# haoyu94/RoITr

Hardware: AMD Instinct MI355X
Metric: point-cloud pairs/s (higher is better)
Workload: dtype f32

## Files before the change

roitr_amd/csrc/pointops_knn.hip:

```cpp
#include "common.h"
#include "knn_grid.h"
#include "prof.h"
#include "roitr_pointops.h"
#include <math.h>
#include <stdio.h>
#include <stdlib.h>
#include <type_traits>

#define KNN_FILL 1e10f

namespace {

__device__ __forceinline__ float rl_f(float v, int lane) { return __int_as_float(__builtin_amdgcn_readlane(__float_as_int(v), lane)); }
__device__ __forceinline__ int rl_i(int v, int lane) { return __builtin_amdgcn_readlane(v, lane); }
__device__ __forceinline__ void lds_sync_wave() { asm volatile("s_waitcnt lgkmcnt(0)" ::: "memory"); }
__device__ __forceinline__ void push_query(int* count, int* list, int q) { list[atomicAdd(count, 1)] = q; }

__device__ __forceinline__ void home_cell(const RoitrGrid& g, float x, float y, float z, int (&c)[3])
{
    c[0] = (int)fminf(fmaxf((x - g.ox) * g.inv_h, 0.f), (float)(g.nx - 1));
    c[1] = (int)fminf(fmaxf((y - g.oy) * g.inv_h, 0.f), (float)(g.ny - 1));
    c[2] = (int)fminf(fmaxf((z - g.oz) * g.inv_h, 0.f), (float)(g.nz - 1));
}
struct ShellBox { int x0, x1, y0, y1, z0, z1; };
// ... 88 lines not shown
        const int p = lane + 64 * r;
        if (p < nsample) {
            if (o.idx) o.idx[(size_t)q * nsample + p] = i[r];
            if (o.dist2) o.dist2[(size_t)q * nsample + p] = d[r];
            if (p >= 1) {
                if (o.group_idx) o.group_idx[(size_t)q * (nsample - 1) + p - 1] = i[r];
                if (o.ppf) {
                    const float* pp = xyz + (size_t)i[r] * 3;
                    const float* pn = o.ref_normals + (size_t)i[r] * 3;
                    const float* qn = o.query_normals + (size_t)q * 3;
                    const float4 f = ppf4(Q.x, Q.y, Q.z, qn[0], qn[1], qn[2], pp[0], pp[1], pp[2], pn[0], pn[1], pn[2]);
                    reinterpret_cast<float4*>(o.ppf)[(size_t)q * (nsample - 1) + p - 1] = f;
                }
            }
        }
    }
}

template <int NR>
__device__ __forceinline__ bool has_tie(const WaveList<NR>& L, int nsample, int lane)
{
    bool t = false;
    float nxt_first = 0.f;
    if (NR > 1) nxt_first = rl_f(L.d[NR - 1], 0);
#pragma unroll
    for (int r = 0; r < NR; ++r) {
        float nx = __shfl_down(L.d[r], 1, 64);
        const int p = lane + 64 * r;
        if (lane == 63) nx = (r + 1 < NR) ? nxt_first : __int_as_float(0x7fc00000);
        t |= (p < nsample) && (L.d[r] == nx) && (L.d[r] < KNN_FILL);
    }
    return __ballot(t) != 0ull;
}

__device__ __forceinline__ void find_segment(int q, const int* __restrict__ offset, const int* __restrict__ new_offset, int& start,
                                             int& end, int& seg, int b = 0)
{
    int bt = 0;
    if (b > 0) bt = segment_of(q, new_offset, b);
    else
    while (!(q < new_offset[bt])) bt++;
    start = bt == 0 ? 0 : offset[bt - 1];
    end = offset[bt];
    seg = bt;
}

template <int NR>
__device__ __forceinline__ void finish_query(WaveList<NR>& L, const KnnOut& o, int q, int nsample, int lane, const float* xyz, Query Q)
{
    if (has_tie(L, nsample, lane)) {
        if (lane == 0) push_query(o.tie_count, o.tie_list, q);
        return;
    }
    write_rows<NR>(o, q, nsample, L.d, L.i, lane, xyz, Q);
}

template <int NR>
__global__ __launch_bounds__(256) void knn_brute_kernel(int m, int nsample, const float* __restrict__ xyz,
                                                        const float* __restrict__ new_xyz, const int* __restrict__ offset,
                                                        const int* __restrict__ new_offset, KnnOut o)
{
    const int lane = threadIdx.x & 63;
    const int q = blockIdx.x * 4 + (threadIdx.x >> 6);
    if (q >= m) return;
    int start, end, seg;
    find_segment(q, offset, new_offset, start, end, seg, o.b);
    Query Q = {new_xyz[(size_t)q * 3], new_xyz[(size_t)q * 3 + 1], new_xyz[(size_t)q * 3 + 2]};
    WaveList<NR> L;
    L.init(start);
    const int tau_pos = nsample;
    float tau = KNN_FILL;
    for (int base = start; base < end; base += 64) {
        const int k = base + lane;
        float cd = INFINITY;
        if (k < end) {
            const float* p = xyz + (size_t)k * 3;
            cd = sqdist3(Q.x, Q.y, Q.z, p[0], p[1], p[2]);
        }
        consume_batch<NR>(L, cd, k, tau, tau_pos, lane);
    }
    finish_query<NR>(L, o, q, nsample, lane, xyz, Q);
}

template <int CAP>
__global__ __launch_bounds__(1024) void grid_build_kernel(const float* __restrict__ xyz, const int* __restrict__ offset,
                                                          RoitrGrid* __restrict__ grids, int* __restrict__ cell_start,
                                                          float4* __restrict__ sorted, float target_occupancy)
{
    __shared__ int cnt[CAP];
    __shared__ float red[6][16];
    __shared__ RoitrGrid G;
    __shared__ int wave_tot[16];
    const int c = blockIdx.x;
    const int start = c == 0 ? 0 : offset[c - 1];
    const int end = offset[c];
    const int n = end - start;
    const int tid = threadIdx.x, lane = tid & 63, wave = tid >> 6;
    int* cs = cell_start + (size_t)c * (GRID_MAX_CELLS + 1);

    float mn[3] = {INFINITY, INFINITY, INFINITY}, mx[3] = {-INFINITY, -INFINITY, -INFINITY};
    for (int k = start + tid; k < end; k += 1024) {
#pragma unroll
        for (int a = 0; a < 3; ++a) {
            const float v = xyz[(size_t)k * 3 + a];
            mn[a] = fminf(mn[a], v); mx[a] = fmaxf(mx[a], v);
        }
    }
#pragma unroll
    for (int a = 0; a < 3; ++a) {
        const float lo = -wave_max(-mn[a]), hi = wave_max(mx[a]);
        if (lane == 0) { red[a][wave] = lo; red[3 + a][wave] = hi; }
    }
    __shared__ int occ_cells;
    __shared__ int refine;
    if (tid == 0) occ_cells = 0;
    __syncthreads();
    auto choose = [&](float h_want) {
        float lo[3], ext[3], me = 0.f;
        for (int a = 0; a < 3; ++a) {
            float l = red[a][0], h = red[3 + a][0];
            for (int w = 1; w < 16; ++w) { l = fminf(l, red[a][w]); h = fmaxf(h, red[3 + a][w]); }
            if (n == 0) { l = 0.f; h = 0.f; }
            lo[a] = l; ext[a] = h - l; me = fmaxf(me, ext[a]);
        }
        if (!(me > 0.f)) me = 1.f;
        float h = h_want;
        if (!(h > 0.f)) {
            float vol = 1.f;
            for (int a = 0; a < 3; ++a) vol *= fmaxf(ext[a], 1e-3f * me);
            h = cbrtf(vol * target_occupancy / (float)(n > 0 ? n : 1));
        }
        h = fmaxf(h, me / (float)GRID_MAX_DIM);
        int d[3];
        for (;;) {
            long tot = 1;
            for (int a = 0; a < 3; ++a) {
                int v = (int)floorf(ext[a] / h) + 1;
                d[a] = v < 1 ? 1 : (v > GRID_MAX_DIM ? GRID_MAX_DIM : v);
                tot *= d[a];
            }
            if (tot <= CAP) break;
            h *= 1.26f;
        }
        G.ox = lo[0]; G.oy = lo[1]; G.oz = lo[2]; G.h = h; G.inv_h = 1.0f / h; G.nx = d[0]; G.ny = d[1]; G.nz = d[2];
    };
    if (tid == 0) choose(0.f);
    __syncthreads();
    for (int k = tid; k < G.nx * G.ny * G.nz; k += 1024) cnt[k] = 0;
    __syncthreads();
    auto cell_of_g = [&](float x, float y, float z) {
        int cx = (int)floorf((x - G.ox) * G.inv_h), cy = (int)floorf((y - G.oy) * G.inv_h), cz = (int)floorf((z - G.oz) * G.inv_h);
        cx = min(max(cx, 0), G.nx - 1); cy = min(max(cy, 0), G.ny - 1); cz = min(max(cz, 0), G.nz - 1);
        return (cz * G.ny + cy) * G.nx + cx;
    };
    for (int pass = 0; pass < 3; ++pass) {
        for (int k = start + tid; k < end; k += 1024)
            atomicAdd(&cnt[cell_of_g(xyz[(size_t)k * 3], xyz[(size_t)k * 3 + 1], xyz[(size_t)k * 3 + 2])], 1);
        __syncthreads();
        if (pass == 2) break;
        const int nc_ = G.nx * G.ny * G.nz;
        int occ_l = 0;
        for (int k = tid; k < nc_; k += 1024) occ_l += cnt[k] > 0 ? 1 : 0;
        occ_l = (int)wave_sum((float)occ_l);
        if (lane == 0 && occ_l) atomicAdd(&occ_cells, occ_l);
        __syncthreads();
        if (tid == 0) {
            const float have = (float)n / (float)max(occ_cells, 1);
            refine = 0;
            if (n > 0 && have > 1.3f * target_occupancy) {
                const float h_old = G.h;
                choose(h_old * cbrtf(target_occupancy / have));
                refine = G.h < 0.97f * h_old ? 1 : 0;
                if (!refine) choose(h_old);
            }
            occ_cells = 0;
        }
        __syncthreads();
        if (!refine) break;
        for (int k = tid; k < G.nx * G.ny * G.nz; k += 1024) cnt[k] = 0;
        __syncthreads();
    }
    if (tid == 0) grids[c] = G;
    const RoitrGrid g = G;
    const int ncell = g.nx * g.ny * g.nz;
    auto cell_of = [&](float x, float y, float z) {
        int cx = (int)floorf((x - g.ox) * g.inv_h), cy = (int)floorf((y - g.oy) * g.inv_h), cz = (int)floorf((z - g.oz) * g.inv_h);
        cx = min(max(cx, 0), g.nx - 1); cy = min(max(cy, 0), g.ny - 1); cz = min(max(cz, 0), g.nz - 1);
        return (cz * g.ny + cy) * g.nx + cx;
    };
    {
        constexpr int PER = CAP / 1024;
        int loc[PER], s = 0;
#pragma unroll
        for (int j = 0; j < PER; ++j) { const int k = tid * PER + j; loc[j] = k < ncell ? cnt[k] : 0; s += loc[j]; }
        int incl = s;
#pragma unroll
        for (int o = 1; o < 64; o <<= 1) { const int v = __shfl_up(incl, o, 64); if (lane >= o) incl += v; }
        if (lane == 63) wave_tot[wave] = incl;
        __syncthreads();
        int wbase = 0;
        for (int w = 0; w < wave; ++w) wbase += wave_tot[w];
        int run = wbase + incl - s;
#pragma unroll
        for (int j = 0; j < PER; ++j) {
            const int k = tid * PER + j;
            if (k < ncell) { cnt[k] = run; cs[k] = start + run; }
            run += loc[j];
        }
        if (tid == 0) cs[ncell] = start + n;
    }
    __syncthreads();
    for (int k = start + tid; k < end; k += 1024) {
        const float x = xyz[(size_t)k * 3], y = xyz[(size_t)k * 3 + 1], z = xyz[(size_t)k * 3 + 2];
        const int pos = atomicAdd(&cnt[cell_of(x, y, z)], 1);
        sorted[start + pos] = make_float4(x, y, z, __int_as_float(k));
    }
}

constexpr int SEL_CAP = 1024;

template <int J>
__device__ __forceinline__ int lane_xor(int v, int lane)
{
    if (J == 1) return __builtin_amdgcn_update_dpp(0, v, 0xB1, 0xf, 0xf, true);
    if (J == 2) return __builtin_amdgcn_update_dpp(0, v, 0x4E, 0xf, 0xf, true);
    if (J == 4) {
        const int dn = __builtin_amdgcn_update_dpp(0, v, 0x124, 0xf, 0xa, false);
        return __builtin_amdgcn_update_dpp(dn, v, 0x12C, 0xf, 0x5, false);
    }
    if (J == 8) return __builtin_amdgcn_update_dpp(0, v, 0x128, 0xf, 0xf, true);
    return __shfl_xor(v, J, 64);
}

template <int K, int J>
__device__ __forceinline__ void sort128_step(WaveList<2>& L, int lane)
{
#pragma unroll
    for (int r = 0; r < 2; ++r) {
        const int e = lane + 64 * r;
        const float pd = __int_as_float(lane_xor<J>(__float_as_int(L.d[r]), lane));
        const int pi = lane_xor<J>(L.i[r], lane);
        const bool up = (e & K) == 0;
        const bool lower = (lane & J) == 0;
        const unsigned long long mk_ = ((unsigned long long)__float_as_uint(L.d[r]) << 32) | (unsigned)L.i[r];
        const unsigned long long pk_ = ((unsigned long long)__float_as_uint(pd) << 32) | (unsigned)pi;
        const bool mine_gt = mk_ > pk_;
        const bool take = (lower == up) ? mine_gt : !mine_gt;
        L.d[r] = take ? pd : L.d[r];
        L.i[r] = take ? pi : L.i[r];
    }
}
template <int K>
__device__ __forceinline__ void sort128_stage(WaveList<2>& L, int lane)
{
    if (K >= 128) {
        const bool sw = (L.d[0] > L.d[1]) || (L.d[0] == L.d[1] && L.i[0] > L.i[1]);
        const float td = sw ? L.d[1] : L.d[0]; const int ti = sw ? L.i[1] : L.i[0];
        L.d[1] = sw ? L.d[0] : L.d[1]; L.i[1] = sw ? L.i[0] : L.i[1];
        L.d[0] = td; L.i[0] = ti;
    }
    if (K >= 64) sort128_step<K, 32>(L, lane);
    if (K >= 32) sort128_step<K, 16>(L, lane);
    if (K >= 16) sort128_step<K, 8>(L, lane);
    if (K >= 8) sort128_step<K, 4>(L, lane);
    if (K >= 4) sort128_step<K, 2>(L, lane);
    sort128_step<K, 1>(L, lane);
}
__device__ __forceinline__ void wave_sort128(WaveList<2>& L, int lane)
{
    sort128_stage<2>(L, lane); sort128_stage<4>(L, lane); sort128_stage<8>(L, lane); sort128_stage<16>(L, lane);
    sort128_stage<32>(L, lane); sort128_stage<64>(L, lane); sort128_stage<128>(L, lane);
}
__global__ __launch_bounds__(256) void knn_gridsel_kernel(int m, int nsample, const float* __restrict__ xyz,
                                                          const float* __restrict__ new_xyz, const int* __restrict__ offset,
                                                          const int* __restrict__ new_offset, const RoitrGrid* __restrict__ grids,
                                                          const int* __restrict__ cell_start, const float4* __restrict__ sorted, KnnOut o,
                                                          const int* __restrict__ qlist, const int* __restrict__ qcount)
{
    __shared__ float bd_[4][SEL_CAP];
    __shared__ int bi_[4][SEL_CAP];
    __shared__ float ld_[4][128];
    __shared__ int li_[4][128];
    __shared__ int hist_[4][64];
    const int lane = threadIdx.x & 63, w = threadIdx.x >> 6;
    const int n_q = qlist ? *qcount : m;
    for (int t_ = blockIdx.x * 4 + w; t_ < n_q; t_ += gridDim.x * 4) {
    const int q = qlist ? qlist[t_] : t_;
    float* bd = bd_[w]; int* bi = bi_[w]; float* ld = ld_[w]; int* li = li_[w]; int* hist = hist_[w];
    int start, end, seg;
    find_segment(q, offset, new_offset, start, end, seg, o.b);
    const RoitrGrid g = grids[seg];
    const int* cs = cell_start + (size_t)seg * (GRID_MAX_CELLS + 1);
    Query Q = {new_xyz[(size_t)q * 3], new_xyz[(size_t)q * 3 + 1], new_xyz[(size_t)q * 3 + 2]};
    WaveList<2> L;
    L.init(start);
    const int need = nsample + 1;
    float tau = KNN_FILL;
    int cnt = 0;
    bool overflow = false, sorted_ok = false;
// ... 291 lines not shown
            const int S1 = S + 1;
            const float hi = lim;
            const float scale = 64.0f / hi;
            hist[lane] = 0;
            lds_sync_wave();
            int bin[4];
#pragma unroll
            for (int r = 0; r < 4; ++r) {
                bin[r] = min(63, (int)(e[r] * scale));
                if (lane + 64 * r < cnt) atomicAdd(&hist[bin[r]], 1);
            }
            lds_sync_wave();
            const int h = hist[lane];
            const int incl = wave_incl_scan(h, lane);
            const unsigned long long ge = __ballot(incl >= S1);
            const int B = __ffsll((long long)ge) - 1;
            const int nB = rl_i(h, B);
            const int r_need = S1 - (rl_i(incl, B) - nB);
            float tau;
            {
                int base = 0;
                bool too_many = false;
#pragma unroll
                for (int r = 0; r < 4; ++r) {
                    const bool inb = (lane + 64 * r < cnt) && bin[r] == B;
                    const unsigned long long mk = __ballot(inb);
                    const int pos = __builtin_amdgcn_mbcnt_hi((unsigned)(mk >> 32), __builtin_amdgcn_mbcnt_lo((unsigned)mk, base));
                    if (inb && pos < 64) sd[pos] = e[r];
                    base += __popcll(mk);
                }
                too_many = base > 64;
                if (too_many) { retry(q); continue; }
                lds_sync_wave();
                const float v = lane < nB ? sd[lane] : INFINITY;
                int rank = 0;
                for (int u = 0; u < nB; ++u) rank += (rl_f(v, u) < v) ? 1 : 0;
                const float tv = (lane < nB && rank < r_need) ? v : -1.0f;
                tau = wave_max(tv);
                const int n_le = __popcll(__ballot(lane < nB && v <= tau));
                if (n_le != r_need) { tie(q); continue; }
            }
            {
                int base = 0;
#pragma unroll
                for (int r = 0; r < 4; ++r) {
                    const bool sel = e[r] <= tau && ej[r] != qslot;
                    const unsigned long long mk = __ballot(sel);
                    const int pos = __builtin_amdgcn_mbcnt_hi((unsigned)(mk >> 32), __builtin_amdgcn_mbcnt_lo((unsigned)mk, base));
                    if (sel && pos < 64) { sd[pos] = e[r]; sj[pos] = ej[r]; }
                    base += __popcll(mk);
                }
                if (base != S) { retry(q); continue; }
            }
            lds_sync_wave();
            float d = lane < S ? sd[lane] : INFINITY;
            int j = lane < S ? sj[lane] : 0;
            wave_sort64(d, j, lane);
            {
                const float nxd = __shfl_down(d, 1, 64);
                const bool t = (lane + 1 < S && d == nxd) || (lane == 0 && d == 0.f);
                if (__ballot(t) != 0ull) { tie(q); continue; }
            }
            const float4 nb = j >= 0 ? cand[j] : sorted[-j - 1];
            const int ni = __float_as_int(nb.w);
            if (lane == 0) {
                if (o.idx) o.idx[(size_t)q * nsample] = q;
                if (o.dist2) o.dist2[(size_t)q * nsample] = 0.f;
            }
            if (lane < S) {
                if (o.idx) o.idx[(size_t)q * nsample + lane + 1] = ni;
                if (o.dist2) o.dist2[(size_t)q * nsample + lane + 1] = d;
                if (o.group_idx) o.group_idx[(size_t)q * S + lane] = ni;
                if (o.ppf) {
                    const float* pn = o.ref_normals + (size_t)ni * 3;
                    const float* qn = o.query_normals + (size_t)q * 3;
                    reinterpret_cast<float4*>(o.ppf)[(size_t)q * S + lane] =
                        ppf4(Qp.x, Qp.y, Qp.z, qn[0], qn[1], qn[2], nb.x, nb.y, nb.z, pn[0], pn[1], pn[2]);
                }
            }
        }
    }
}

template <int CAP>
__global__ __launch_bounds__(1024) void sort_queries_kernel(const float* __restrict__ new_xyz, const int* __restrict__ new_offset,
                                                            const RoitrGrid* __restrict__ grids, int* __restrict__ qorder)
{
    __shared__ int cnt[CAP];
    __shared__ int wave_tot[16];
    const int c = blockIdx.x;
    const int start = c == 0 ? 0 : new_offset[c - 1], end = new_offset[c];
    const int tid = threadIdx.x, lane = tid & 63, wave = tid >> 6;
    const RoitrGrid g = grids[c];
    const int ncell = g.nx * g.ny * g.nz;
    auto cell_of = [&](int k) {
        int c0[3];
        home_cell(g, new_xyz[(size_t)k * 3], new_xyz[(size_t)k * 3 + 1], new_xyz[(size_t)k * 3 + 2], c0);
        return (c0[2] * g.ny + c0[1]) * g.nx + c0[0];
    };
    for (int k = tid; k < ncell; k += 1024) cnt[k] = 0;
    __syncthreads();
    for (int k = start + tid; k < end; k += 1024) atomicAdd(&cnt[cell_of(k)], 1);
    __syncthreads();
    constexpr int PER = CAP / 1024;
    int loc[PER], sum = 0;
#pragma unroll
    for (int j = 0; j < PER; ++j) { const int k = tid * PER + j; loc[j] = k < ncell ? cnt[k] : 0; sum += loc[j]; }
    int incl = sum;
#pragma unroll
    for (int o = 1; o < 64; o <<= 1) { const int v = __shfl_up(incl, o, 64); if (lane >= o) incl += v; }
    if (lane == 63) wave_tot[wave] = incl;
    __syncthreads();
    int run = incl - sum;
    for (int w = 0; w < wave; ++w) run += wave_tot[w];
#pragma unroll
    for (int j = 0; j < PER; ++j) { const int k = tid * PER + j; if (k < ncell) cnt[k] = run; run += loc[j]; }
    __syncthreads();
    for (int k = start + tid; k < end; k += 1024) qorder[start + atomicAdd(&cnt[cell_of(k)], 1)] = k;
}

template <int L>
__device__ __forceinline__ void lane_emit(const KnnOut& o, int q, int nsample, const float (&d)[L], const int (&id)[L], bool tie,
                                          const float* __restrict__ xyz, float qx, float qy, float qz)
{
    if (tie) {
        push_query(o.tie_count, o.tie_list, q);
        return;
    }
#pragma unroll
    for (int j = 0; j < L; ++j) {
        if (j < nsample) {
            if (o.idx) o.idx[(size_t)q * nsample + j] = id[j];
            if (o.dist2) o.dist2[(size_t)q * nsample + j] = d[j];
            if (j >= 1 && o.group_idx) o.group_idx[(size_t)q * (nsample - 1) + j - 1] = id[j];
        }
    }
    if (o.ppf) {
        const float* qn = o.query_normals + (size_t)q * 3;
        const float nx = qn[0], ny = qn[1], nz = qn[2];
        for (int j = 0; j < nsample - 1; ++j) {
            const int gi = o.group_idx[(size_t)q * (nsample - 1) + j];
            const float* pp = xyz + (size_t)gi * 3;
            const float* pn = o.ref_normals + (size_t)gi * 3;
            reinterpret_cast<float4*>(o.ppf)[(size_t)q * (nsample - 1) + j] =
                ppf4(qx, qy, qz, nx, ny, nz, pp[0], pp[1], pp[2], pn[0], pn[1], pn[2]);
        }
    }
}

template <int L, int CAP>
__global__ __launch_bounds__(256) void knn_prefilter_kernel(int m, int nsample, int b, const float* __restrict__ xyz,
                                                            const float* __restrict__ new_xyz, const int* __restrict__ offset,
                                                            const int* __restrict__ new_offset, const RoitrGrid* __restrict__ grids,
                                                            const int* __restrict__ cell_start, const float4* __restrict__ sorted, KnnOut o,
                                                            int self_sorted, const int* __restrict__ qorder, int* __restrict__ retry_count,
                                                            int* __restrict__ retry_list)
{
    __shared__ int surv[CAP][256];
    const int nblk = (m + 255) >> 8;
    const int blk = xcd_block_id(nblk);
    if (blk >= nblk) return;
    const int tid = threadIdx.x;
    const int t = blk * 256 + tid;
    if (t >= m) return;
    const int q = self_sorted ? __float_as_int(sorted[t].w) : (qorder ? qorder[t] : t);
    const int seg = segment_of(q, new_offset, b);
    const int start = seg == 0 ? 0 : offset[seg - 1];
    const RoitrGrid g = grids[seg];
    const int* cs = cell_start + (size_t)seg * (GRID_MAX_CELLS + 1);
    const float qx = new_xyz[(size_t)q * 3], qy = new_xyz[(size_t)q * 3 + 1], qz = new_xyz[(size_t)q * 3 + 2];
    int c0[3];
    home_cell(g, qx, qy, qz, c0);
    const ShellBox B = shell_box(c0, 1, g);
    const int x0 = B.x0, x1 = B.x1, y0 = B.y0, y1 = B.y1, z0 = B.z0, z1 = B.z1;
    const float dm = unseen_bound(g, B, qx, qy, qz) - 2e-4f * g.h;
    int nbox = 0;
    for (int cz = z0; cz <= z1; ++cz)
        for (int cy = y0; cy <= y1; ++cy) {
            const int rowbase = (cz * g.ny + cy) * g.nx;
            nbox += cs[rowbase + x1 + 1] - cs[rowbase + x0];
        }
    const float vbox = (float)((x1 - x0 + 1) * (y1 - y0 + 1) * (z1 - z0 + 1)) * g.h * g.h * g.h;
    const float want = fmaxf(2.0f * (float)(nsample + 1), (float)(nsample + 9));
    const float r0 = cbrtf(want * vbox * 0.2387324f / (float)max(nbox, 1));
    const float fd[6] = {qx - g.ox, g.ox + (float)g.nx * g.h - qx, qy - g.oy, g.oy + (float)g.ny * g.h - qy, qz - g.oz, g.oz + (float)g.nz * g.h - qz};
    float r_est = r0;
#pragma unroll
    for (int itr = 0; itr < 2; ++itr) {
        float inside = 1.0f;
#pragma unroll
        for (int f = 0; f < 6; ++f) {
            const float hc = r_est - fmaxf(fd[f], 0.f);
            if (hc > 0.f) inside -= hc * hc * (3.0f * r_est - hc) / (4.0f * r_est * r_est * r_est);
        }
        r_est = r0 * rcbrtf(fmaxf(inside, 0.125f));
    }
    const float tau = dm > 0.f ? fminf(dm, r_est) : 0.f;
    const float tau2 = tau * tau;
    int cnt = 0;
    for (int cz = z0; cz <= z1; ++cz)
        for (int cy = y0; cy <= y1; ++cy) {
// ... 376 lines not shown
    l.retry = l.qorder + (size_t)m;
    l.end = l.retry + (size_t)m;
    return l;
}

struct WsView {
    int* tie_count; int* tie_list; RoitrGrid* grids; int* cell_start; float4* sorted; int* qorder; int* retry;
};
WsView carve(void* ws, int b, int n, int m)
{
    int* p = (int*)(((uintptr_t)ws + 15) & ~(uintptr_t)15);
    const KnnLayout l = knn_layout(b, n, m);
    const bool grid = b > 0 && n > 0;
    return WsView{p, p + l.tie_list, (RoitrGrid*)(p + l.grids), p + l.cell_start, (float4*)(p + l.sorted), grid ? p + l.qorder : nullptr,
                  grid ? p + l.retry : nullptr};
}

int knn_grid_cap(int b, int n) { return (long)n <= 6144L * b ? 4096 : GRID_MAX_CELLS; }

struct KnnPlan { int form; int width; int sort_cap; };

int lane_width(int need) { return need <= 2 ? 2 : need <= 4 ? 4 : need <= 10 ? 10 : need <= 18 ? 18 : 34; }
template <class F>
void with_lane_width(int width, F f)
{
    switch (width) {
    case 2: f(std::integral_constant<int, 2>()); break;
    case 4: f(std::integral_constant<int, 4>()); break;
    case 10: f(std::integral_constant<int, 10>()); break;
    case 18: f(std::integral_constant<int, 18>()); break;
    default: f(std::integral_constant<int, 34>());
    }
}

int knn_plan(int b, int n, int m, int nsample, bool self, int outputs, bool normals, bool use_grid, float cap2, KnnPlan* p)
{
    *p = KnnPlan{ROITR_KNN_NOTHING, 0, 0};
    if (m <= 0) return ROITR_OK;
    if (nsample < 1 || nsample > 100) return ROITR_ERR_ARG;
    const bool ppf = outputs & ROITR_KNN_OUT_PPF, group = outputs & ROITR_KNN_OUT_GROUP;
    if (ppf && !normals) return ROITR_ERR_ARG;
    constexpr int lane_min = 8192, lane_brute_min = 65536;
    const int need = nsample + 1;
    const bool has_lists = b > 0 && n > 0;
    const bool lane_ok = use_grid && m >= lane_min && (!ppf || group) && b > 0;
    if (lane_ok && !self && has_lists) p->sort_cap = knn_grid_cap(b, n);
    if (lane_ok && need <= 34) {
        p->width = lane_width(need);
        if (cap2 < INFINITY && nsample == 1 && outputs == ROITR_KNN_OUT_DIST2) { p->form = ROITR_KNN_WITHIN; p->width = 0; }
        else p->form = (need > 4 && need <= 10 && cap2 == INFINITY && has_lists) ? ROITR_KNN_PREFILTER : ROITR_KNN_LANE;
    } else if (use_grid && self && has_lists && nsample - 1 <= 64) p->form = ROITR_KNN_CELL;
    else if (use_grid) p->form = ROITR_KNN_GRIDSEL;
    else if (need <= 34 && (!ppf || group) && m >= lane_brute_min) { p->form = ROITR_KNN_LANE_BRUTE; p->width = lane_width(need); }
    else { p->form = ROITR_KNN_BRUTE; p->width = need <= 64 ? 1 : 2; }
    return ROITR_OK;
}
}

extern "C" int roitr_knn_form(int b, int n, int m, int nsample, int self_query, int outputs, int normals, int use_grid, int capped)
{
    KnnPlan p;
    const int st = knn_plan(b, n, m, nsample, self_query != 0, outputs, normals != 0, use_grid != 0, capped ? 1.0f : INFINITY, &p);
    if (st != ROITR_OK) return -st;
    const int sort = p.sort_cap == 0 ? ROITR_KNN_SORT_NONE : p.sort_cap == 4096 ? ROITR_KNN_SORT_4096 : ROITR_KNN_SORT_MAX;
    return p.form | p.width << 8 | sort << 16;
}

extern "C" size_t roitr_knn_workspace_bytes(int b, int n, int m) { return knn_layout(b, n, m).end * 4 + 64; }

extern "C" int roitr_knn_build_grid_ex(int b, int n, int m_capacity, const float* xyz, const int* offset, void* ws, float target_occupancy,
                                       hipStream_t stream);
extern "C" int roitr_knn_build_grid(int b, int n, int m_capacity, const float* xyz, const int* offset, void* ws, hipStream_t stream)
{
    return roitr_knn_build_grid_ex(b, n, m_capacity, xyz, offset, ws, 0.f, stream);
}

extern "C" int roitr_knn_build_grid_ex(int b, int n, int m_capacity, const float* xyz, const int* offset, void* ws, float target_occupancy,
                                       hipStream_t stream)
{
    if (b <= 0 || n <= 0) return ROITR_OK;
    WsView v = carve(ws, b, n, m_capacity);
    const float rho = target_occupancy > 0.f ? target_occupancy : 6.0f;
    roitr_prof_begin(ROITR_PROF_GRID, 12.0 * n + 16.0 * n, stream);
    if (knn_grid_cap(b, n) == 4096) grid_build_kernel<4096><<<b, 1024, 0, stream>>>(xyz, offset, v.grids, v.cell_start, v.sorted, rho);
    else grid_build_kernel<GRID_MAX_CELLS><<<b, 1024, 0, stream>>>(xyz, offset, v.grids, v.cell_start, v.sorted, rho);
    roitr_prof_end(ROITR_PROF_GRID, stream);
    ROITR_LAUNCH_CHECK();
    return ROITR_OK;
}

extern "C" const void* roitr_knn_sorted_points(int b, int n, int m_capacity, void* ws)
{
    return carve(ws, b, n, m_capacity).sorted;
}

RoitrGridView roitr_knn_grid_view(int b, int n, int m_capacity, void* ws)
{
    const WsView v = carve(ws, b, n, m_capacity);
    return RoitrGridView{v.grids, v.cell_start, v.sorted};
}

namespace {
int knnquery_impl(int b, int n, int m, int nsample, const float* xyz, const float* new_xyz, const int* offset,
                  const int* new_offset, int* idx, float* dist2, int* group_idx, float* ppf,
                  const float* ref_normals, const float* query_normals, int use_grid, int m_capacity, void* ws,
                  float cap2, hipStream_t stream)
{
    const int self_sorted = (new_xyz == xyz && new_offset == offset && m == n) ? 1 : 0;
    const int outputs = (idx ? ROITR_KNN_OUT_IDX : 0) | (dist2 ? ROITR_KNN_OUT_DIST2 : 0) | (group_idx ? ROITR_KNN_OUT_GROUP : 0) | (ppf ? ROITR_KNN_OUT_PPF : 0);
    KnnPlan p;
    const int st = knn_plan(b, n, m, nsample, self_sorted != 0, outputs, ref_normals && query_normals, use_grid != 0, cap2, &p);
    if (st != ROITR_OK || p.form == ROITR_KNN_NOTHING) return st;
    WsView v = carve(ws, b, n, m_capacity);
    KnnOut o = {idx, dist2, group_idx, ppf, ref_normals, query_normals, v.tie_count, v.tie_list, b > 0 ? b : 0};
    ROITR_HIP(hipMemsetAsync(v.tie_count, 0, 2 * sizeof(int), stream));
    int* const retry_count = v.tie_count + 1;
    {
        const int kk = group_idx || ppf ? nsample - 1 : nsample;
        double bytes = (ppf ? 24.0 : 12.0) * n + (new_xyz != xyz ? (ppf ? 24.0 : 12.0) * m : 0.0);
        bytes += ((idx ? 4.0 * nsample : 0.0) + (dist2 ? 4.0 * nsample : 0.0) + (group_idx ? 4.0 * kk : 0.0) + (ppf ? 16.0 * kk : 0.0)) * m;
        roitr_prof_begin(ROITR_PROF_KNN, bytes, stream);
    }
    int* qorder = nullptr;
    if (p.sort_cap) {
        qorder = v.qorder;
        if (p.sort_cap == 4096) sort_queries_kernel<4096><<<b, 1024, 0, stream>>>(new_xyz, new_offset, v.grids, qorder);
        else sort_queries_kernel<GRID_MAX_CELLS><<<b, 1024, 0, stream>>>(new_xyz, new_offset, v.grids, qorder);
    }
    const int wave_blocks = div_up(m, 4), lane_blocks = div_up(m, 256);
    switch (p.form) {
    case ROITR_KNN_WITHIN:
        knn_within_kernel<<<xcd_grid(lane_blocks), 256, 0, stream>>>(m, b, new_xyz, new_offset, v.grids, v.cell_start, v.sorted, qorder, cap2, dist2);
        break;
    case ROITR_KNN_LANE:
        with_lane_width(p.width, [&](auto L) {
            knn_lane_kernel<decltype(L)::value><<<xcd_grid(lane_blocks), 256, 0, stream>>>(
                m, nsample, b, xyz, new_xyz, offset, new_offset, v.grids, v.cell_start, v.sorted, o, self_sorted, qorder, cap2, nullptr, nullptr);
        });
        break;
    case ROITR_KNN_PREFILTER:
        knn_prefilter_kernel<10, 40><<<xcd_grid(lane_blocks), 256, 0, stream>>>(m, nsample, b, xyz, new_xyz, offset, new_offset, v.grids, v.cell_start,
                                                                               v.sorted, o, self_sorted, qorder, retry_count, v.retry);
        knn_lane_kernel<10><<<min(lane_blocks, 1024), 256, 0, stream>>>(m, nsample, b, xyz, new_xyz, offset, new_offset, v.grids, v.cell_start, v.sorted, o,
                                                                        self_sorted, qorder, cap2, v.retry, retry_count);
        break;
    case ROITR_KNN_CELL:
        knn_cell_kernel<<<dim3(1024, b), 256, 0, stream>>>(nsample, xyz, offset, v.grids, v.cell_start, v.sorted, o, retry_count, v.qorder);
        knn_gridsel_kernel<<<1024, 256, 0, stream>>>(m, nsample, xyz, new_xyz, offset, new_offset, v.grids, v.cell_start, v.sorted, o, v.qorder,
                                                      retry_count);
        break;
    case ROITR_KNN_GRIDSEL:
        knn_gridsel_kernel<<<min(wave_blocks, 65536), 256, 0, stream>>>(m, nsample, xyz, new_xyz, offset, new_offset, v.grids, v.cell_start, v.sorted, o,
                                                                         nullptr, nullptr);
        break;
    case ROITR_KNN_LANE_BRUTE: {
        int ch = b > 0 ? (int)(((long)n / b + 63) / 64 * 64) : 1024;
        ch = ch < 64 ? 64 : (ch > 1024 ? 1024 : ch);
        with_lane_width(p.width, [&](auto L) {
            knn_lane_brute_kernel<decltype(L)::value><<<div_up(m, 64), 64, (size_t)ch * 16, stream>>>(m, nsample, b, xyz, new_xyz, offset, new_offset, o, ch);
        });
        break;
    }
    default:
        if (p.width == 1) knn_brute_kernel<1><<<wave_blocks, 256, 0, stream>>>(m, nsample, xyz, new_xyz, offset, new_offset, o);
        else knn_brute_kernel<2><<<wave_blocks, 256, 0, stream>>>(m, nsample, xyz, new_xyz, offset, new_offset, o);
    }
    roitr_prof_end(ROITR_PROF_KNN, stream);
    ROITR_LAUNCH_CHECK();
    roitr_prof_begin(ROITR_PROF_REPLAY, 0.0, stream);
    knn_replay_kernel<<<min(m, 1024), 64, 0, stream>>>(nsample, xyz, new_xyz, offset, new_offset, o);
    roitr_prof_end(ROITR_PROF_REPLAY, stream);
    ROITR_LAUNCH_CHECK();
    {
        struct Stats {
            bool on = getenv("ROITR_KNN_STATS") != nullptr; long q = 0, ties = 0, retries = 0, calls = 0;
            ~Stats() { if (on) fprintf(stderr, "KNNSTATS calls %ld queries %ld replayed %ld cell->general %ld\n", calls, q, ties, retries); }
        };
        static Stats st;
        if (st.on) {
            int h[2] = {0, 0};
            ROITR_HIP(hipMemcpyAsync(h, v.tie_count, sizeof(h), hipMemcpyDeviceToHost, stream));
            ROITR_HIP(hipStreamSynchronize(stream));
            st.calls++; st.q += m; st.ties += h[0]; st.retries += h[1];
        }
    }
    return ROITR_OK;
}
}

extern "C" int roitr_knnquery_ex(int b, int n, int m, int nsample, const float* xyz, const float* new_xyz, const int* offset,
                                 const int* new_offset, int* idx, float* dist2, int* group_idx, float* ppf,
                                 const float* ref_normals, const float* query_normals, int use_grid, int m_capacity, void* ws,
                                 hipStream_t stream)
{
    return knnquery_impl(b, n, m, nsample, xyz, new_xyz, offset, new_offset, idx, dist2, group_idx, ppf, ref_normals, query_normals, use_grid,
                         m_capacity, ws, INFINITY, stream);
}

extern "C" void knnquery_cuda_launcher(int m, int nsample, const float* xyz, const float* new_xyz, const int* offset,
                                       const int* new_offset, int* idx, float* dist2)
{
    if (m <= 0) return;
    const size_t need = (size_t)m + 16;
    if (need > g_legacy_ws_ints) {
        if (g_legacy_ws) (void)hipFree(g_legacy_ws);
        g_legacy_ws_ints = need * 2;
        if (hipMalloc(&g_legacy_ws, g_legacy_ws_ints * sizeof(int)) != hipSuccess) {
            roitr_set_error("hipMalloc failed (legacy knn scratch)", __FILE__, __LINE__);
            g_legacy_ws = nullptr; g_legacy_ws_ints = 0;
            return;
// ... 14 lines not shown
```

Baseline: 6658.

## Hold grid-build points in registers and cache cell ids across passes

```diff
diff --git a/roitr_amd/csrc/pointops_knn.hip b/roitr_amd/csrc/pointops_knn.hip
--- a/roitr_amd/csrc/pointops_knn.hip
+++ b/roitr_amd/csrc/pointops_knn.hip
@@ -194,44 +194,138 @@
     finish_query<NR>(L, o, q, nsample, lane, xyz, Q);
 }
 
-template <int CAP>
+constexpr int GRID_PTS = 24;
+template <int CAP> constexpr int grid_threads = CAP <= 4096 ? 256 : 1024;
+
+struct CellRegs {
+    unsigned v[GRID_PTS / 2];
+    __device__ __forceinline__ void set(int j, int cell) { v[j >> 1] = (j & 1) ? (v[j >> 1] | (unsigned)cell << 16) : (unsigned)cell; }
+    __device__ __forceinline__ int get(int j) const { return (j & 1) ? (int)(v[j >> 1] >> 16) : (int)(v[j >> 1] & 0xffffu); }
+};
+static_assert(GRID_MAX_CELLS <= 65536 && GRID_PTS % 2 == 0, "two cells per register");
+struct P3 { float x, y, z; };
+__device__ __forceinline__ P3 load_p3(const float* __restrict__ pts, int k)
+{
+    P3 p;
+    __builtin_memcpy(&p, pts + (size_t)k * 3, sizeof(P3));
+    return p;
+}
+template <int NT>
+__device__ __forceinline__ int held_point(int j) { return 4 * ((j >> 2) * NT + (int)threadIdx.x) + (j & 3); }
+template <int NT>
+__device__ __forceinline__ bool held(int j, int nh) { return held_point<NT>(j & ~3) < nh; }
+template <int NT>
+__device__ __forceinline__ int held_count(int n) { return min(n, GRID_PTS * NT) & ~3; }
+template <int NT, class F>
+__device__ __forceinline__ void for_held_quads(int nh, F f)
+{
+#pragma unroll
+    for (int g = 0; g < GRID_PTS / 4; ++g)
+        if (held<NT>(4 * g, nh)) f(g, held_point<NT>(4 * g));
+}
+template <int NT>
+__device__ __forceinline__ void load_quad(const float* __restrict__ pts, int g, int nh, float (&f)[12])
+{
+    if (held<NT>(4 * g, nh)) __builtin_memcpy(f, pts + (size_t)held_point<NT>(4 * g) * 3, 48);
+}
+template <int NT, class F>
+__device__ __forceinline__ void stream_points(const float* __restrict__ pts, int from, int n, F f)
+{
+    constexpr int NF = 4;
+    for (int k0 = from + (int)threadIdx.x; k0 < n; k0 += NF * NT) {
+        P3 p[NF];
+#pragma unroll
+        for (int u = 0; u < NF; ++u) p[u] = load_p3(pts, min(k0 + u * NT, n - 1));
+#pragma unroll
+        for (int u = 0; u < NF; ++u)
+            if (k0 + u * NT < n) f(k0 + u * NT, p[u]);
+    }
+}
+__device__ __forceinline__ void clear_cells_all(int* cnt, int cap, int nt)
+{
+    for (int k = threadIdx.x; k < cap / 4; k += nt) reinterpret_cast<int4*>(cnt)[k] = make_int4(0, 0, 0, 0);
+}
+__device__ __forceinline__ RoitrGrid uniform_grid(const RoitrGrid& s)
+{
+    const auto uf = [](float v) { return __int_as_float(__builtin_amdgcn_readfirstlane(__float_as_int(v))); };
+    const auto ui = [](int v) { return __builtin_amdgcn_readfirstlane(v); };
+    return RoitrGrid{uf(s.ox), uf(s.oy), uf(s.oz), uf(s.h), uf(s.inv_h), ui(s.nx), ui(s.ny), ui(s.nz)};
+}
+template <int CAP, int NT>
+__device__ __forceinline__ void cell_scan(int* cnt, int* wave_tot)
+{
+    constexpr int PER4 = CAP / NT / 4;
+    static_assert(CAP % (4 * NT) == 0, "whole int4 per thread");
+    const int tid = threadIdx.x, lane = tid & 63, wave = tid >> 6;
+    int4* c4 = reinterpret_cast<int4*>(cnt) + tid * PER4;
+    int s = 0;
+#pragma unroll
+    for (int i = 0; i < PER4; ++i) { const int4 v = c4[i]; s += v.x + v.y + v.z + v.w; }
+    int incl = s;
+#pragma unroll
+    for (int o = 1; o < 64; o <<= 1) { const int v = __shfl_up(incl, o, 64); if (lane >= o) incl += v; }
+    if (lane == 63) wave_tot[wave] = incl;
+    __syncthreads();
+    int run = incl - s;
+    for (int w = 0; w < wave; ++w) run += wave_tot[w];
+#pragma unroll
+    for (int i = 0; i < PER4; ++i) {
+        const int4 v = c4[i];
+        int4 e;
+        e.x = run; run += v.x; e.y = run; run += v.y; e.z = run; run += v.z; e.w = run; run += v.w;
+        c4[i] = e;
+    }
+    __syncthreads();
+}
+
+template <int CAP, int NT>
 __global__ __launch_bounds__(1024) void grid_build_kernel(const float* __restrict__ xyz, const int* __restrict__ offset,
-                                                          RoitrGrid* __restrict__ grids, int* __restrict__ cell_start,
-                                                          float4* __restrict__ sorted, float target_occupancy)
-{
-    __shared__ int cnt[CAP];
-    __shared__ float red[6][16];
+                                                        RoitrGrid* __restrict__ grids, int* __restrict__ cell_start,
+                                                        float4* __restrict__ sorted, float target_occupancy)
+{
+    constexpr int NW = NT / 64;
+    __shared__ __attribute__((aligned(16))) int cnt[CAP];
+    __shared__ float red[6][NW];
     __shared__ RoitrGrid G;
-    __shared__ int wave_tot[16];
+    __shared__ int wave_tot[NW];
+    __shared__ int occ_cells;
+    __shared__ int refine;
     const int c = blockIdx.x;
     const int start = c == 0 ? 0 : offset[c - 1];
     const int end = offset[c];
     const int n = end - start;
+    const int nh = held_count<NT>(n);
     const int tid = threadIdx.x, lane = tid & 63, wave = tid >> 6;
+    const float* __restrict__ cloud = xyz + (size_t)start * 3;
     int* cs = cell_start + (size_t)c * (GRID_MAX_CELLS + 1);
 
+    float pt[GRID_PTS / 4][12];
+#pragma unroll
+    for (int g = 0; g < GRID_PTS / 4; ++g) load_quad<NT>(cloud, g, nh, pt[g]);
+    clear_cells_all(cnt, CAP, NT);
+    if (tid == 0) occ_cells = 0;
+
     float mn[3] = {INFINITY, INFINITY, INFINITY}, mx[3] = {-INFINITY, -INFINITY, -INFINITY};
-    for (int k = start + tid; k < end; k += 1024) {
-#pragma unroll
-        for (int a = 0; a < 3; ++a) {
-            const float v = xyz[(size_t)k * 3 + a];
-            mn[a] = fminf(mn[a], v); mx[a] = fmaxf(mx[a], v);
-        }
-    }
+    for_held_quads<NT>(nh, [&](int g, int) {
+#pragma unroll
+        for (int i = 0; i < 12; ++i) { mn[i % 3] = fminf(mn[i % 3], pt[g][i]); mx[i % 3] = fmaxf(mx[i % 3], pt[g][i]); }
+    });
+    stream_points<NT>(cloud, nh, n, [&](int, const P3& p) {
+        mn[0] = fminf(mn[0], p.x); mx[0] = fmaxf(mx[0], p.x);
+        mn[1] = fminf(mn[1], p.y); mx[1] = fmaxf(mx[1], p.y);
+        mn[2] = fminf(mn[2], p.z); mx[2] = fmaxf(mx[2], p.z);
+    });
 #pragma unroll
     for (int a = 0; a < 3; ++a) {
         const float lo = -wave_max(-mn[a]), hi = wave_max(mx[a]);
         if (lane == 0) { red[a][wave] = lo; red[3 + a][wave] = hi; }
     }
-    __shared__ int occ_cells;
-    __shared__ int refine;
-    if (tid == 0) occ_cells = 0;
     __syncthreads();
     auto choose = [&](float h_want) {
         float lo[3], ext[3], me = 0.f;
         for (int a = 0; a < 3; ++a) {
             float l = red[a][0], h = red[3 + a][0];
-            for (int w = 1; w < 16; ++w) { l = fminf(l, red[a][w]); h = fmaxf(h, red[3 + a][w]); }
+            for (int w = 1; w < NW; ++w) { l = fminf(l, red[a][w]); h = fmaxf(h, red[3 + a][w]); }
             if (n == 0) { l = 0.f; h = 0.f; }
             lo[a] = l; ext[a] = h - l; me = fmaxf(me, ext[a]);
         }
@@ -258,21 +352,28 @@
     };
     if (tid == 0) choose(0.f);
     __syncthreads();
-    for (int k = tid; k < G.nx * G.ny * G.nz; k += 1024) cnt[k] = 0;
-    __syncthreads();
-    auto cell_of_g = [&](float x, float y, float z) {
-        int cx = (int)floorf((x - G.ox) * G.inv_h), cy = (int)floorf((y - G.oy) * G.inv_h), cz = (int)floorf((z - G.oz) * G.inv_h);
-        cx = min(max(cx, 0), G.nx - 1); cy = min(max(cy, 0), G.ny - 1); cz = min(max(cz, 0), G.nz - 1);
-        return (cz * G.ny + cy) * G.nx + cx;
+    auto cell_of = [](const RoitrGrid& g, float x, float y, float z) {
+        int cx = (int)floorf((x - g.ox) * g.inv_h), cy = (int)floorf((y - g.oy) * g.inv_h), cz = (int)floorf((z - g.oz) * g.inv_h);
+        cx = min(max(cx, 0), g.nx - 1); cy = min(max(cy, 0), g.ny - 1); cz = min(max(cz, 0), g.nz - 1);
+        return (cz * g.ny + cy) * g.nx + cx;
     };
+    CellRegs cell;
     for (int pass = 0; pass < 3; ++pass) {
-        for (int k = start + tid; k < end; k += 1024)
-            atomicAdd(&cnt[cell_of_g(xyz[(size_t)k * 3], xyz[(size_t)k * 3 + 1], xyz[(size_t)k * 3 + 2])], 1);
+        const RoitrGrid g = uniform_grid(G);
+        for_held_quads<NT>(nh, [&](int q, int) {
+#pragma unroll
+            for (int u = 0; u < 4; ++u) {
+                const int cj = cell_of(g, pt[q][3 * u], pt[q][3 * u + 1], pt[q][3 * u + 2]);
+                cell.set(4 * q + u, cj);
+                atomicAdd(&cnt[cj], 1);
+            }
+        });
+        stream_points<NT>(cloud, nh, n, [&](int, const P3& p) { atomicAdd(&cnt[cell_of(g, p.x, p.y, p.z)], 1); });
         __syncthreads();
         if (pass == 2) break;
-        const int nc_ = G.nx * G.ny * G.nz;
+        const int nc_ = g.nx * g.ny * g.nz;
         int occ_l = 0;
-        for (int k = tid; k < nc_; k += 1024) occ_l += cnt[k] > 0 ? 1 : 0;
+        for (int k = tid; k < nc_; k += NT) occ_l += cnt[k] > 0 ? 1 : 0;
         occ_l = (int)wave_sum((float)occ_l);
         if (lane == 0 && occ_l) atomicAdd(&occ_cells, occ_l);
         __syncthreads();
@@ -289,44 +390,27 @@
         }
         __syncthreads();
         if (!refine) break;
-        for (int k = tid; k < G.nx * G.ny * G.nz; k += 1024) cnt[k] = 0;
+        for (int k = tid; k < nc_; k += NT) cnt[k] = 0;
         __syncthreads();
     }
     if (tid == 0) grids[c] = G;
-    const RoitrGrid g = G;
+    const RoitrGrid g = uniform_grid(G);
     const int ncell = g.nx * g.ny * g.nz;
-    auto cell_of = [&](float x, float y, float z) {
-        int cx = (int)floorf((x - g.ox) * g.inv_h), cy = (int)floorf((y - g.oy) * g.inv_h), cz = (int)floorf((z - g.oz) * g.inv_h);
-        cx = min(max(cx, 0), g.nx - 1); cy = min(max(cy, 0), g.ny - 1); cz = min(max(cz, 0), g.nz - 1);
-        return (cz * g.ny + cy) * g.nx + cx;
-    };
-    {
-        constexpr int PER = CAP / 1024;
-        int loc[PER], s = 0;
-#pragma unroll
-        for (int j = 0; j < PER; ++j) { const int k = tid * PER + j; loc[j] = k < ncell ? cnt[k] : 0; s += loc[j]; }
-        int incl = s;
-#pragma unroll
-        for (int o = 1; o < 64; o <<= 1) { const int v = __shfl_up(incl, o, 64); if (lane >= o) incl += v; }
-        if (lane == 63) wave_tot[wave] = incl;
-        __syncthreads();
-        int wbase = 0;
-        for (int w = 0; w < wave; ++w) wbase += wave_tot[w];
-        int run = wbase + incl - s;
-#pragma unroll
-        for (int j = 0; j < PER; ++j) {
-            const int k = tid * PER + j;
-            if (k < ncell) { cnt[k] = run; cs[k] = start + run; }
-            run += loc[j];
-        }
-        if (tid == 0) cs[ncell] = start + n;
-    }
+    cell_scan<CAP, NT>(cnt, wave_tot);
+    for_held_quads<NT>(nh, [&](int q, int k4) {
+#pragma unroll
+        for (int u = 0; u < 4; ++u) {
+            const int pos = atomicAdd(&cnt[cell.get(4 * q + u)], 1);
+            sorted[start + pos] = make_float4(pt[q][3 * u], pt[q][3 * u + 1], pt[q][3 * u + 2], __int_as_float(start + k4 + u));
+        }
+    });
+    stream_points<NT>(cloud, nh, n, [&](int k, const P3& p) {
+        const int pos = atomicAdd(&cnt[cell_of(g, p.x, p.y, p.z)], 1);
+        sorted[start + pos] = make_float4(p.x, p.y, p.z, __int_as_float(start + k));
+    });
     __syncthreads();
-    for (int k = start + tid; k < end; k += 1024) {
-        const float x = xyz[(size_t)k * 3], y = xyz[(size_t)k * 3 + 1], z = xyz[(size_t)k * 3 + 2];
-        const int pos = atomicAdd(&cnt[cell_of(x, y, z)], 1);
-        sorted[start + pos] = make_float4(x, y, z, __int_as_float(k));
-    }
+    if (tid == 0) cs[0] = start;
+    for (int k = tid; k < ncell; k += NT) cs[k + 1] = start + cnt[k];
 }
 
 constexpr int SEL_CAP = 1024;
@@ -784,41 +868,47 @@
     }
 }
 
-template <int CAP>
-__global__ __launch_bounds__(1024) void sort_queries_kernel(const float* __restrict__ new_xyz, const int* __restrict__ new_offset,
-                                                            const RoitrGrid* __restrict__ grids, int* __restrict__ qorder)
-{
-    __shared__ int cnt[CAP];
-    __shared__ int wave_tot[16];
+template <int CAP, int NT>
+__global__ __launch_bounds__(NT) void sort_queries_kernel(const float* __restrict__ new_xyz, const int* __restrict__ new_offset,
+                                                          const RoitrGrid* __restrict__ grids, int* __restrict__ qorder)
+{
+    constexpr int NW = NT / 64;
+    __shared__ __attribute__((aligned(16))) int cnt[CAP];
+    __shared__ int wave_tot[NW];
     const int c = blockIdx.x;
     const int start = c == 0 ? 0 : new_offset[c - 1], end = new_offset[c];
-    const int tid = threadIdx.x, lane = tid & 63, wave = tid >> 6;
-    const RoitrGrid g = grids[c];
-    const int ncell = g.nx * g.ny * g.nz;
-    auto cell_of = [&](int k) {
+    const int m = end - start, mh = held_count<NT>(m);
+    const float* __restrict__ queries = new_xyz + (size_t)start * 3;
+    const RoitrGrid g = uniform_grid(grids[c]);
+    auto cell_of = [&](const P3& p) {
         int c0[3];
-        home_cell(g, new_xyz[(size_t)k * 3], new_xyz[(size_t)k * 3 + 1], new_xyz[(size_t)k * 3 + 2], c0);
+        home_cell(g, p.x, p.y, p.z, c0);
         return (c0[2] * g.ny + c0[1]) * g.nx + c0[0];
     };
-    for (int k = tid; k < ncell; k += 1024) cnt[k] = 0;
+    CellRegs cell;
+    {
+        float f[GRID_PTS / 4][12];
+#pragma unroll
+        for (int q4 = 0; q4 < GRID_PTS / 4; ++q4) load_quad<NT>(queries, q4, mh, f[q4]);
+        for_held_quads<NT>(mh, [&](int q4, int) {
+#pragma unroll
+            for (int u = 0; u < 4; ++u) cell.set(4 * q4 + u, cell_of(P3{f[q4][3 * u], f[q4][3 * u + 1], f[q4][3 * u + 2]}));
+        });
+    }
+    clear_cells_all(cnt, CAP, NT);
     __syncthreads();
-    for (int k = start + tid; k < end; k += 1024) atomicAdd(&cnt[cell_of(k)], 1);
+    for_held_quads<NT>(mh, [&](int q4, int) {
+#pragma unroll
+        for (int u = 0; u < 4; ++u) atomicAdd(&cnt[cell.get(4 * q4 + u)], 1);
+    });
+    stream_points<NT>(queries, mh, m, [&](int, const P3& p) { atomicAdd(&cnt[cell_of(p)], 1); });
     __syncthreads();
-    constexpr int PER = CAP / 1024;
-    int loc[PER], sum = 0;
-#pragma unroll
-    for (int j = 0; j < PER; ++j) { const int k = tid * PER + j; loc[j] = k < ncell ? cnt[k] : 0; sum += loc[j]; }
-    int incl = sum;
-#pragma unroll
-    for (int o = 1; o < 64; o <<= 1) { const int v = __shfl_up(incl, o, 64); if (lane >= o) incl += v; }
-    if (lane == 63) wave_tot[wave] = incl;
-    __syncthreads();
-    int run = incl - sum;
-    for (int w = 0; w < wave; ++w) run += wave_tot[w];
-#pragma unroll
-    for (int j = 0; j < PER; ++j) { const int k = tid * PER + j; if (k < ncell) cnt[k] = run; run += loc[j]; }
-    __syncthreads();
-    for (int k = start + tid; k < end; k += 1024) qorder[start + atomicAdd(&cnt[cell_of(k)], 1)] = k;
+    cell_scan<CAP, NT>(cnt, wave_tot);
+    for_held_quads<NT>(mh, [&](int q4, int k4) {
+#pragma unroll
+        for (int u = 0; u < 4; ++u) qorder[start + atomicAdd(&cnt[cell.get(4 * q4 + u)], 1)] = start + k4 + u;
+    });
+    stream_points<NT>(queries, mh, m, [&](int k, const P3& p) { qorder[start + atomicAdd(&cnt[cell_of(p)], 1)] = start + k; });
 }
 
 template <int L>
@@ -1361,8 +1451,12 @@
     WsView v = carve(ws, b, n, m_capacity);
     const float rho = target_occupancy > 0.f ? target_occupancy : 6.0f;
     roitr_prof_begin(ROITR_PROF_GRID, 12.0 * n + 16.0 * n, stream);
-    if (knn_grid_cap(b, n) == 4096) grid_build_kernel<4096><<<b, 1024, 0, stream>>>(xyz, offset, v.grids, v.cell_start, v.sorted, rho);
-    else grid_build_kernel<GRID_MAX_CELLS><<<b, 1024, 0, stream>>>(xyz, offset, v.grids, v.cell_start, v.sorted, rho);
+    const auto launch = [&](auto cap) {
+        constexpr int CAP = decltype(cap)::value, NT = grid_threads<CAP>;
+        grid_build_kernel<CAP, NT><<<b, NT, 0, stream>>>(xyz, offset, v.grids, v.cell_start, v.sorted, rho);
+    };
+    if (knn_grid_cap(b, n) == 4096) launch(std::integral_constant<int, 4096>());
+    else launch(std::integral_constant<int, GRID_MAX_CELLS>());
     roitr_prof_end(ROITR_PROF_GRID, stream);
     ROITR_LAUNCH_CHECK();
     return ROITR_OK;
@@ -1403,8 +1497,12 @@
     int* qorder = nullptr;
     if (p.sort_cap) {
         qorder = v.qorder;
-        if (p.sort_cap == 4096) sort_queries_kernel<4096><<<b, 1024, 0, stream>>>(new_xyz, new_offset, v.grids, qorder);
-        else sort_queries_kernel<GRID_MAX_CELLS><<<b, 1024, 0, stream>>>(new_xyz, new_offset, v.grids, qorder);
+        const auto launch = [&](auto cap) {
+            constexpr int CAP = decltype(cap)::value, NT = grid_threads<CAP>;
+            sort_queries_kernel<CAP, NT><<<b, NT, 0, stream>>>(new_xyz, new_offset, v.grids, qorder);
+        };
+        if (p.sort_cap == 4096) launch(std::integral_constant<int, 4096>());
+        else launch(std::integral_constant<int, GRID_MAX_CELLS>());
     }
     const int wave_blocks = div_up(m, 4), lane_blocks = div_up(m, 256);
     switch (p.form) {
```

Result: no change. 6634 (-0.4%).
